# dbolya/yolact

Hardware: NVIDIA H100
Metric: frames/sec @ 550x550 yolact_base (Yolact.forward + Detect + postprocess) (higher is better)
Workload: dtype f16x3 (fp16 hi+lo operand pairs, 3 wgmma passes, fp32 accumulate: fp32-equivalent, parity-tested at 1e-3)

## Files before the change

yolact_b200/csrc/tc_common.cuh:

```cuda
#pragma once
#include <cuda.h>
#include "kernels.cuh"

namespace yb {
namespace tc {

__device__ __forceinline__ uint32_t smem_u32(const void* p) {
  return (uint32_t)__cvta_generic_to_shared(p);
}
__device__ __forceinline__ void mbar_init(uint64_t* bar, uint32_t count) {
  asm volatile("mbarrier.init.shared::cta.b64 [%0], %1;" ::"r"(smem_u32(bar)), "r"(count));
}
__device__ __forceinline__ void mbar_expect_tx(uint64_t* bar, uint32_t bytes) {
  asm volatile("mbarrier.arrive.expect_tx.shared::cta.b64 _, [%0], %1;" ::"r"(smem_u32(bar)), "r"(bytes)
               : "memory");
}
__device__ __forceinline__ bool mbar_try_wait(uint32_t addr, uint32_t parity) {
  uint32_t ok;
  asm volatile(
      "{\n\t"
      ".reg .pred P1;\n\t"
      "mbarrier.try_wait.parity.shared::cta.b64 P1, [%1], %2;\n\t"
      "selp.u32 %0, 1, 0, P1;\n\t"
      "}"
      : "=r"(ok)
      : "r"(addr), "r"(parity)
      : "memory");
  return ok != 0;
}
__device__ __forceinline__ bool mbar_test_wait(uint32_t addr, uint32_t parity) {
  uint32_t ok;
  asm volatile(
      "{\n\t"
      ".reg .pred P1;\n\t"
      "mbarrier.test_wait.parity.shared::cta.b64 P1, [%1], %2;\n\t"
      "selp.u32 %0, 1, 0, P1;\n\t"
      "}"
      : "=r"(ok)
      : "r"(addr), "r"(parity)
      : "memory");
  return ok != 0;
}
__device__ __forceinline__ void mbar_arrive(uint64_t* bar) {
  asm volatile("mbarrier.arrive.shared::cta.b64 _, [%0];" ::"r"(smem_u32(bar)) : "memory");
}
__device__ __forceinline__ void mbar_wait(uint64_t* bar, uint32_t parity) {
  const uint32_t addr = smem_u32(bar);
#ifndef YB_WATCHDOG
  while (!mbar_try_wait(addr, parity)) {
  }
#else
  if (mbar_try_wait(addr, parity)) return;
  const long long t0 = clock64();
  while (!mbar_try_wait(addr, parity)) {
    if (clock64() - t0 > 4000000000ll) asm volatile("trap;");
  }
#endif
}
__device__ __forceinline__ void fence_barrier_init() {
  asm volatile("fence.mbarrier_init.release.cluster;" ::: "memory");
}
__device__ __forceinline__ void tma_prefetch_desc(const void* desc) {
  asm volatile("prefetch.tensormap [%0];" ::"l"(reinterpret_cast<uint64_t>(desc)) : "memory");
}
__device__ __forceinline__ void tma_load_4d(void* smem_dst, const void* desc, uint64_t* bar, int c0,
                                            int c1, int c2, int c3) {
  asm volatile(
      "cp.async.bulk.tensor.4d.shared::cluster.global.mbarrier::complete_tx::bytes"
      " [%0], [%1, {%3, %4, %5, %6}], [%2];" ::"r"(smem_u32(smem_dst)),
      "l"(reinterpret_cast<uint64_t>(desc)), "r"(smem_u32(bar)), "r"(c0), "r"(c1), "r"(c2), "r"(c3)
      : "memory");
}
__device__ __forceinline__ void tma_load_3d(void* smem_dst, const void* desc, uint64_t* bar, int c0,
                                            int c1, int c2) {
  asm volatile(
      "cp.async.bulk.tensor.3d.shared::cluster.global.mbarrier::complete_tx::bytes"
      " [%0], [%1, {%3, %4, %5}], [%2];" ::"r"(smem_u32(smem_dst)),
      "l"(reinterpret_cast<uint64_t>(desc)), "r"(smem_u32(bar)), "r"(c0), "r"(c1), "r"(c2)
      : "memory");
}
__device__ __forceinline__ void tma_store_4d(const void* desc, const void* smem_src, int c0, int c1, int c2, int c3) {
  asm volatile("cp.async.bulk.tensor.4d.global.shared::cta.bulk_group [%0, {%2, %3, %4, %5}], [%1];" ::"l"(
                   reinterpret_cast<uint64_t>(desc)),
               "r"(smem_u32(smem_src)), "r"(c0), "r"(c1), "r"(c2), "r"(c3)
               : "memory");
}
__device__ __forceinline__ void bulk_commit() { asm volatile("cp.async.bulk.commit_group;" ::: "memory"); }
template <int N>
__device__ __forceinline__ void bulk_wait_read() {
  asm volatile("cp.async.bulk.wait_group.read %0;" ::"n"(N) : "memory");
}
__device__ __forceinline__ void bulk_wait_all() { asm volatile("cp.async.bulk.wait_group 0;" ::: "memory"); }
__device__ __forceinline__ void fence_proxy_async() { asm volatile("fence.proxy.async.shared::cta;" ::: "memory"); }
__device__ __forceinline__ void fence_proxy_async_all() { asm volatile("fence.proxy.async;" ::: "memory"); }
__device__ __forceinline__ int ld_acquire_gpu(const int* p) {
  int v;
  asm volatile("ld.acquire.gpu.global.s32 %0, [%1];" : "=r"(v) : "l"(p) : "memory");
  return v;
}
__device__ __forceinline__ void st_release_gpu(int* p, int v) {
  asm volatile("st.release.gpu.global.s32 [%0], %1;" ::"l"(p), "r"(v) : "memory");
}
__device__ __forceinline__ void st_relaxed_gpu(int* p, int v) {
  asm volatile("st.relaxed.gpu.global.s32 [%0], %1;" ::"l"(p), "r"(v) : "memory");
}
__device__ __forceinline__ void red_release_gpu_add(int* p, int v) {
  asm volatile("red.release.gpu.global.add.s32 [%0], %1;" ::"l"(p), "r"(v) : "memory");
}
__device__ __forceinline__ uint4 ldg_nc16(const void* p) {
  uint4 r;
  asm volatile("ld.global.nc.v4.u32 {%0, %1, %2, %3}, [%4];" : "=r"(r.x), "=r"(r.y), "=r"(r.z), "=r"(r.w) : "l"(p));
  return r;
}
__device__ __forceinline__ uint32_t cluster_ctarank() {
  uint32_t r;
  asm volatile("mov.u32 %0, %%cluster_ctarank;" : "=r"(r));
  return r;
}
__device__ __forceinline__ uint32_t cluster_id_x() {
  uint32_t r;
  asm volatile("mov.u32 %0, %%clusterid.x;" : "=r"(r));
  return r;
}
__device__ __forceinline__ uint32_t cluster_nclusters_x() {
  uint32_t r;
  asm volatile("mov.u32 %0, %%nclusterid.x;" : "=r"(r));
  return r;
}
__device__ __forceinline__ void cluster_sync_all() {
  asm volatile("barrier.cluster.arrive.release.aligned;" ::: "memory");
  asm volatile("barrier.cluster.wait.acquire.aligned;" ::: "memory");
}
__device__ __forceinline__ uint32_t mapa_u32(uint32_t smem_cta_addr, uint32_t rank) {
  uint32_t r;
  asm volatile("mapa.shared::cluster.u32 %0, %1, %2;" : "=r"(r) : "r"(smem_cta_addr), "r"(rank));
  return r;
}
__device__ __forceinline__ void mbar_arrive_cluster(uint32_t cluster_addr) {
  asm volatile("mbarrier.arrive.release.cluster.shared::cluster.b64 _, [%0];" ::"r"(cluster_addr) : "memory");
}
__device__ __forceinline__ void tma_load_3d_mc(void* smem_dst, const void* desc, uint64_t* bar, uint16_t mask, int c0, int c1,
                                               int c2) {
  asm volatile(
      "cp.async.bulk.tensor.3d.shared::cluster.global.mbarrier::complete_tx::bytes.multicast::cluster"
      " [%0], [%1, {%3, %4, %5}], [%2], %6;" ::"r"(smem_u32(smem_dst)),
      "l"(reinterpret_cast<uint64_t>(desc)), "r"(smem_u32(bar)), "r"(c0), "r"(c1), "r"(c2), "h"(mask)
      : "memory");
}

__device__ __forceinline__ void wgmma_fence() { asm volatile("wgmma.fence.sync.aligned;" ::: "memory"); }
__device__ __forceinline__ void wgmma_commit() { asm volatile("wgmma.commit_group.sync.aligned;" ::: "memory"); }
template <int N>
__device__ __forceinline__ void wgmma_wait() {
  asm volatile("wgmma.wait_group.sync.aligned %0;" ::"n"(N) : "memory");
}
template <int R>
__device__ __forceinline__ void fence_regs(float* d) {
#pragma unroll
  for (int i = 0; i < R; ++i) asm volatile("" : "+f"(d[i])::"memory");
}
template <int N>
struct Wgmma;
template <>
struct Wgmma<32> {
  __device__ __forceinline__ static void mma(float* d, uint64_t da, uint64_t db, uint32_t scale_d) {
    asm volatile(
        "{\n\t"
        ".reg .pred p;\n\t"
        "setp.ne.b32 p, %18, 0;\n\t"
        "wgmma.mma_async.sync.aligned.m64n32k16.f32.f16.f16 "
        "{"
        "%0, %1, %2, %3, %4, %5, %6, %7, %8, %9, %10, %11, %12, %13, %14, %15 "
        "}, %16, %17, p, 1, 1, 0, 0;\n\t"
        "}"
        : "+f"(d[0]), "+f"(d[1]), "+f"(d[2]), "+f"(d[3]), "+f"(d[4]), "+f"(d[5]), "+f"(d[6]), "+f"(d[7]),
          "+f"(d[8]), "+f"(d[9]), "+f"(d[10]), "+f"(d[11]), "+f"(d[12]), "+f"(d[13]), "+f"(d[14]), "+f"(d[15])
        : "l"(da), "l"(db), "r"(scale_d));
  }
};
template <>
struct Wgmma<64> {
  __device__ __forceinline__ static void mma(float* d, uint64_t da, uint64_t db, uint32_t scale_d) {
    asm volatile(
        "{\n\t"
        ".reg .pred p;\n\t"
        "setp.ne.b32 p, %34, 0;\n\t"
        "wgmma.mma_async.sync.aligned.m64n64k16.f32.f16.f16 "
        "{"
// ... 117 lines not shown
```

yolact_b200/csrc/tc_conv.cu:

```cuda
#include <atomic>
#include <vector>
#include "tc_common.cuh"

namespace yb {

using namespace tc;

namespace {

constexpr int BLOCK_M = 128;
constexpr int BLOCK_K = 64;
constexpr int A_STAGE_BYTES = BLOCK_M * BLOCK_K * 2;
constexpr int MAX_TAPS = 9;
constexpr int MAX_STAGES = 8;

struct alignas(64) TcParams {
  CUtensorMap tmA[4];
  CUtensorMap tmB;
  CUtensorMap tmY;
  CUtensorMap tmR;
  int epi_tma;
  int out_off;
  int res_off;
  int m_tiles, n_tiles;
// ... 3 lines not shown
  float* seg_y[3];
  int pdl;
  int pair;
  int nb;
  int ntaps, kchunks, stages;
  int tap_map[MAX_TAPS], tap_dx[MAX_TAPS], tap_dy[MAX_TAPS];
  int tw, th, tiles_x, tiles_y;
  int Ho, Wo, Cout;
  int a_box_bytes;
  void* y;
  const float* bias;
  const __half* residual;
  long long y_batch_stride;
  long long res_batch_stride;
  int y_pix_stride;
  int y_f32;
  int act;
  int vec_ok;
  int res_after_act;
  int split;
  int cin;
  float out_scale;
  int sk;
  float* sk_ws;
  int* sk_flags;
  int res_direct;
  int bn;
};

__device__ __forceinline__ void mma_bar_sync(int nthreads) { asm volatile("bar.sync 1, %0;" ::"r"(nthreads) : "memory"); }

template <int BN, int MH, int H, bool SPLIT, bool PAIR, int NACC>
__device__ __forceinline__ void mma_tile(float (&acc)[MH][SPLIT ? 2 : 1][NACC], uint8_t* smem, uint64_t* full_bar,
                                         uint64_t* empty_bar, int stages, int stage_bytes, int a_bytes, int b_plane_bytes,
                                         uint32_t& kbg, int nkb, int cw, bool signaller) {
  constexpr int NPL = SPLIT ? 2 : 1;
#pragma unroll
  for (int mh = 0; mh < MH; ++mh)
#pragma unroll
    for (int pl = 0; pl < NPL; ++pl)
#pragma unroll
      for (int i = 0; i < BN / 2; ++i) acc[mh][pl][i] = 0.f;
  auto release = [&](uint32_t s) {
    if (!signaller) return;
    if (PAIR) {
      mbar_arrive_cluster(mapa_u32(smem_u32(&empty_bar[s]), 0));
      mbar_arrive_cluster(mapa_u32(smem_u32(&empty_bar[s]), 1));
    } else {
      mbar_arrive(&empty_bar[s]);
    }
  };
  for (int kb = 0; kb < nkb; ++kb, ++kbg) {
    const uint32_t s = kbg % (uint32_t)stages;
    mbar_wait(&full_bar[s], (kbg / (uint32_t)stages) & 1u);
    const uint32_t sa = smem_u32(smem + (size_t)s * stage_bytes);
    const uint32_t sb = sa + (uint32_t)a_bytes;
    wgmma_fence();
#pragma unroll
    for (int mh = 0; mh < MH; ++mh) {
      const uint32_t half_off = (uint32_t)(cw + mh * H) * (64u * 128u);
      mma_passes<BN, BLOCK_K / 16, SPLIT>(
          acc[mh][0], acc[mh][NPL - 1],
          [&](int pl, int k) { return make_sw128_desc(sa + (uint32_t)(pl * A_STAGE_BYTES) + half_off) + (uint64_t)(2 * k); },
          [&](int pl, int k) { return make_sw128_desc(sb + (uint32_t)(pl * b_plane_bytes)) + (uint64_t)(2 * k); });
    }
    wgmma_commit();
    if (stages == 1) {
      wgmma_wait<0>();
      release(s);
    } else if (kb > 0) {
      wgmma_wait<1>();
      release((kbg - 1) % (uint32_t)stages);
    }
  }
  wgmma_wait<0>();
  if (nkb > 0 && stages > 1) release((kbg - 1) % (uint32_t)stages);
#pragma unroll
  for (int mh = 0; mh < MH; ++mh)
#pragma unroll
    for (int pl = 0; pl < NPL; ++pl) fence_regs<BN / 2>(acc[mh][pl]);
  if (SPLIT) {
#pragma unroll
    for (int mh = 0; mh < MH; ++mh)
#pragma unroll
      for (int i = 0; i < BN / 2; ++i) acc[mh][0][i] = split_combine(acc[mh][0][i], acc[mh][NPL - 1][i]);
  }
}

struct EpiArgs {
  const CUtensorMap* tmY;
  const CUtensorMap* tmR;
  uint64_t* res_full_bar;
  uint8_t* out_base;
  uint8_t* res_base;
  const float* bias;
  const __half* res_g;
  int res_pix_stride;
  uint32_t res_tx;
  int Wo, Cout, n0, x0, y0, b, nchunks, nbuf;
  float out_scale;
};
template <int ACT, bool RES_AFTER, bool SPLIT, int BN, int MH, int H, int NACC>
__device__ __forceinline__ void epi_staged(float (&acc)[MH][SPLIT ? 2 : 1][NACC], const EpiArgs& e, bool has_res_tile,
                                           uint32_t& g, int cw, int ct, int lane, int wq) {
  constexpr int NPL = SPLIT ? 2 : 1;
  const int nthreads = 128 * H;
#pragma unroll
  for (int c = 0; c < BN / 64; ++c) {
    if (c >= e.nchunks) break;
    const uint32_t buf = (e.nbuf == 1) ? 0u : (g & 1u);
    uint8_t* out_tile = e.out_base + buf * (NPL * A_STAGE_BYTES);
    const uint8_t* res_tile = e.res_base + buf * (NPL * A_STAGE_BYTES);
    if (g >= (uint32_t)e.nbuf) {
      if (ct == 0) {
        if (e.nbuf == 1) bulk_wait_read<0>(); else bulk_wait_read<1>();
      }
      mma_bar_sync(nthreads);
    }
    if (has_res_tile) {
      if (ct == 0 && e.nbuf == 2 && c + 1 < e.nchunks) {
        const uint32_t nb = (g + 1) & 1u;
        mbar_expect_tx(&e.res_full_bar[nb], e.res_tx);
#pragma unroll
        for (int pl = 0; pl < NPL; ++pl)
          tma_load_4d(e.res_base + nb * (NPL * A_STAGE_BYTES) + pl * A_STAGE_BYTES, e.tmR, &e.res_full_bar[nb],
                      e.n0 + (c + 1) * 64 + pl * e.Cout, e.x0, e.y0, e.b);
      }
      mbar_wait(&e.res_full_bar[buf], (e.nbuf == 1) ? (g & 1u) : ((g >> 1) & 1u));
    }
    const int nbase = e.n0 + c * 64;
#pragma unroll
    for (int j = 0; j < 8; ++j) {
      const int col = 8 * j + 2 * (lane & 3);
      const float b0 = (e.bias && nbase + col < e.Cout) ? __ldg(e.bias + nbase + col) : 0.f;
      const float b1 = (e.bias && nbase + col + 1 < e.Cout) ? __ldg(e.bias + nbase + col + 1) : 0.f;
#pragma unroll
      for (int mh = 0; mh < MH; ++mh)
#pragma unroll
        for (int h = 0; h < 2; ++h) {
          const int row = (cw + mh * H) * 64 + wq * 16 + (lane >> 2) + 8 * h;
          const int i = (c * 8 + j) * 4 + 2 * h;
          float v0 = scale_bias<SPLIT>(acc[mh][0][i], e.out_scale, b0);
          float v1 = scale_bias<SPLIT>(acc[mh][0][i + 1], e.out_scale, b1);
          if (RES_AFTER) {
            v0 = act_t<ACT>(v0);
            v1 = act_t<ACT>(v1);
          }
          const uint32_t off = sw128_off((uint32_t)row, (uint32_t)j) + (uint32_t)(lane & 3) * 4u;
          if (has_res_tile || e.res_g) {
            __half2 rh, rl;
            if (has_res_tile) {
              rh = *reinterpret_cast<const __half2*>(res_tile + off);
              if (SPLIT) rl = *reinterpret_cast<const __half2*>(res_tile + A_STAGE_BYTES + off);
            } else if (e.x0 + row < e.Wo) {
              const __half* rp = e.res_g + (size_t)row * e.res_pix_stride + c * 64 + col;
              const unsigned int u = __ldcg(reinterpret_cast<const unsigned int*>(rp));
              rh = *reinterpret_cast<const __half2*>(&u);
              if (SPLIT) {
                const unsigned int ul = __ldcg(reinterpret_cast<const unsigned int*>(rp + e.Cout));
                rl = *reinterpret_cast<const __half2*>(&ul);
              }
            } else {
              rh = rl = __floats2half2_rn(0.f, 0.f);
            }
            const float2 f = __half22float2(rh);
            v0 += f.x;
            v1 += f.y;
            if (SPLIT) {
              const float2 fl = lo2_to_f32(rl);
              v0 += fl.x;
              v1 += fl.y;
            }
          }
          if (!RES_AFTER) {
            v0 = act_t<ACT>(v0);
            v1 = act_t<ACT>(v1);
          }
          __half2 hi, lo;
          if (SPLIT) split2_from_f32(v0, v1, hi, lo);
          else hi = f16x2_from_f32(v0, v1);
          *reinterpret_cast<__half2*>(out_tile + off) = hi;
          if (SPLIT) *reinterpret_cast<__half2*>(out_tile + A_STAGE_BYTES + off) = lo;
        }
    }
    fence_proxy_async();
    mma_bar_sync(nthreads);
    if (ct == 0) {
      tma_store_4d(e.tmY, out_tile, nbase, e.x0, e.y0, e.b);
      if (SPLIT) tma_store_4d(e.tmY, out_tile + A_STAGE_BYTES, nbase + e.Cout, e.x0, e.y0, e.b);
      bulk_commit();
      if (has_res_tile && e.nbuf == 1 && c + 1 < e.nchunks) {
        mbar_expect_tx(&e.res_full_bar[0], e.res_tx);
#pragma unroll
        for (int pl = 0; pl < NPL; ++pl)
          tma_load_4d(e.res_base + pl * A_STAGE_BYTES, e.tmR, &e.res_full_bar[0], e.n0 + (c + 1) * 64 + pl * e.Cout, e.x0,
                      e.y0, e.b);
      }
    }
    ++g;
  }
}

template <bool SPLIT, int BN, int MH, int H, int NACC>
__device__ __forceinline__ void epi_staged_act(int act, int raa, float (&acc)[MH][SPLIT ? 2 : 1][NACC], const EpiArgs& e,
                                               bool has_res_tile, uint32_t& g, int cw, int ct, int lane, int wq) {
  switch (act) {
    case ACT_RELU: epi_staged<ACT_RELU, false, SPLIT, BN, MH, H>(acc, e, has_res_tile, g, cw, ct, lane, wq); break;
    case ACT_LEAKY:
      if (raa) epi_staged<ACT_LEAKY, true, SPLIT, BN, MH, H>(acc, e, has_res_tile, g, cw, ct, lane, wq);
      else epi_staged<ACT_LEAKY, false, SPLIT, BN, MH, H>(acc, e, has_res_tile, g, cw, ct, lane, wq);
      break;
    case ACT_TANH: epi_staged<ACT_TANH, false, SPLIT, BN, MH, H>(acc, e, has_res_tile, g, cw, ct, lane, wq); break;
    default: epi_staged<ACT_NONE, false, SPLIT, BN, MH, H>(acc, e, has_res_tile, g, cw, ct, lane, wq); break;
  }
}

struct TileCoord {
  int b, x0, y0, n0;
};
__device__ __forceinline__ TileCoord decode_mn(const TcParams& p, int m, int nt, int BN) {
  TileCoord t;
  const int tx = m % p.tiles_x;
  m /= p.tiles_x;
  const int ty = m % p.tiles_y;
  t.b = m / p.tiles_y;
  t.x0 = tx * p.tw;
  t.y0 = ty * p.th;
  t.n0 = nt * BN;
  return t;
}
template <bool PAIR>
__device__ __forceinline__ TileCoord decode_unit(const TcParams& p, int u, int rank, int BN) {
  const int nt = u % p.n_tiles;
  const int mg = u / p.n_tiles;
  return decode_mn(p, PAIR ? 2 * mg + rank : mg, nt, BN);
}

struct WorkIter {
  int num_kb, num_units, ustep, sk, u;
  long long it, it_hi;
  __device__ __forceinline__ static long long share_lo(long long total, int c, int G) { return total * c / G; }
  __device__ __forceinline__ void init(int sk_, int num_kb_, int num_units_, int unit0, int ustep_) {
    sk = sk_;
    num_kb = num_kb_;
    num_units = num_units_;
    ustep = ustep_;
    u = unit0;
    const long long total = (long long)num_units_ * num_kb_;
    it = share_lo(total, unit0, ustep_);
    it_hi = share_lo(total, unit0 + 1, ustep_);
  }
  __device__ __forceinline__ bool next(int& uu, int& k0, int& k1) {
    if (!sk) {
      if (u >= num_units) return false;
      uu = u;
      k0 = 0;
      k1 = num_kb;
      u += ustep;
      return true;
    }
    if (it >= it_hi) return false;
    uu = (int)(it / num_kb);
    k0 = (int)(it - (long long)uu * num_kb);
    const long long rem = it_hi - it;
    k1 = (rem < (long long)(num_kb - k0)) ? (int)(k0 + rem) : num_kb;
    it += k1 - k0;
    return true;
  }
};

template <int BN, bool PAIR, int H, bool SPLIT>
__global__ void __launch_bounds__(128 * (1 + H), 1)
tc_conv_kernel(const __grid_constant__ TcParams p) {
  constexpr int NPL = SPLIT ? 2 : 1;
  constexpr int MH = 2 / H;
  constexpr int NACC = BN / 2;
  static_assert(MH * NPL * NACC <= 128, "accumulator tile exceeds the register budget");
  constexpr int B_PLANE_BYTES = BN * BLOCK_K * 2;
  constexpr int A_BYTES = NPL * A_STAGE_BYTES;
  constexpr int STAGE_BYTES = A_BYTES + NPL * B_PLANE_BYTES;

  extern __shared__ uint8_t smem_dyn[];
  __shared__ uint64_t full_bar[MAX_STAGES];
  __shared__ uint64_t empty_bar[MAX_STAGES];
  __shared__ uint64_t res_full_bar[2];

  uint8_t* smem = reinterpret_cast<uint8_t*>((reinterpret_cast<uintptr_t>(smem_dyn) + 1023) & ~(uintptr_t)1023);

  const int warp = threadIdx.x >> 5;
  const int lane = threadIdx.x & 31;
  const int stages = p.stages;
  const int num_kb = p.ntaps * p.kchunks;
  const int rank = PAIR ? (int)cluster_ctarank() : 0;
  const int unit0 = PAIR ? (int)cluster_id_x() : (int)blockIdx.x;
  const int ustep = PAIR ? (int)cluster_nclusters_x() : (int)gridDim.x;
  const int num_units = (PAIR ? (p.m_tiles + 1) / 2 : p.m_tiles) * p.n_tiles;

  if (threadIdx.x == 0) {
    for (int s = 0; s < stages; ++s) {
      mbar_init(&full_bar[s], 1);
      mbar_init(&empty_bar[s], (PAIR ? 2 : 1) * H);
    }
    for (int i = 0; i < 2; ++i) mbar_init(&res_full_bar[i], 1);
    fence_barrier_init();
    tma_prefetch_desc(&p.tmB);
    tma_prefetch_desc(&p.tmA[0]);
    if (p.epi_tma) tma_prefetch_desc(&p.tmY);
  }
  __syncthreads();
  if (PAIR) cluster_sync_all();
  uint32_t pre = 0;
  if (p.pdl) {
    asm volatile("griddepcontrol.launch_dependents;" ::: "memory");
    if (!PAIR && !SPLIT && !p.sk && threadIdx.x == 0 && unit0 < num_units) {
      const TileCoord t0 = decode_unit<PAIR>(p, unit0, rank, BN);
      const int npre = min(stages, num_kb);
// ... 119 lines not shown
        e.out_base = out_base;
        e.res_base = res_base;
        e.bias = p.bias;
        e.res_g = (p.res_direct && p.residual) ? p.residual + (size_t)x0 * (size_t)(NPL * p.Cout) + n0 : nullptr;
        e.res_pix_stride = NPL * p.Cout;
        e.res_tx = (uint32_t)p.a_box_bytes * (uint32_t)NPL;
        e.Wo = p.Wo;
        e.Cout = p.Cout;
        e.n0 = n0;
        e.x0 = x0;
        e.y0 = y0;
        e.b = b;
        e.nchunks = nchunks;
        e.nbuf = nbuf;
        e.out_scale = p.out_scale;
        epi_staged_act<SPLIT, BN, MH, H>(p.act, p.res_after_act, acc, e, has_res_tile, g, cw, ct, lane, wq);
      } else {
        const int ncols = min(BN, p.Cout - n0);
        const int raa = p.res_after_act;
#pragma unroll
        for (int j = 0; j < BN / 8; ++j) {
          if (8 * j >= ncols) break;
#pragma unroll
          for (int e2 = 0; e2 < 2; ++e2) {
            const int cl = 8 * j + 2 * (lane & 3) + e2;
            if (cl >= ncols) continue;
            const int n = n0 + cl;
            const float bias_n = p.bias ? __ldg(p.bias + n) : 0.f;
            int act = p.act;
            float* seg_base = nullptr;
            long long seg_bs = 0;
            int seg_ps = 0, seg_c = 0;
            if (p.nseg > 0) {
#pragma unroll
              for (int sg = 0; sg < 3; ++sg)
                if (sg < p.nseg && n >= p.seg_begin[sg] && n < p.seg_end[sg]) {
                  seg_base = p.seg_y[sg];
                  seg_bs = p.seg_bs[sg];
                  seg_ps = p.seg_ps[sg];
                  seg_c = n - p.seg_begin[sg];
                  act = p.seg_act[sg];
                }
            }
#pragma unroll
            for (int mh = 0; mh < MH; ++mh)
#pragma unroll
              for (int h = 0; h < 2; ++h) {
                const int trow = (cw + mh * H) * 64 + wq * 16 + (lane >> 2) + 8 * h;
                const int ty_ = trow / p.tw, tx_ = trow - ty_ * p.tw;
                const int oy = y0 + ty_, ox = x0 + tx_;
                if (trow >= p.tw * p.th || oy >= p.Ho || ox >= p.Wo || b >= p.nb) continue;
                const long long pix = (long long)oy * p.Wo + ox;
                const float a = acc[mh][0][j * 4 + 2 * h + e2];
                float v = scale_bias<SPLIT>(a, p.out_scale, bias_n);
                float rsd = 0.f;
                if (p.residual) {
                  const __half* rp = p.residual + ((long long)b * p.res_batch_stride + pix * p.Cout) * NPL + n;
                  rsd = SPLIT ? split_to_f32(rp[0], rp[p.Cout]) : __half2float(rp[0]);
                }
                if (!raa) v += rsd;
                v = apply_act(v, act);
                if (raa) v += rsd;
                if (p.nseg > 0) {
                  if (seg_base) seg_base[(long long)b * seg_bs + pix * seg_ps + seg_c] = v;
                  continue;
                }
                const long long o = (long long)b * p.y_batch_stride + pix * p.y_pix_stride + n;
                if (p.y_f32) {
                  reinterpret_cast<float*>(p.y)[o] = v;
                } else if (SPLIT) {
                  __half hi, lo;
                  split_f32(v, hi, lo);
                  reinterpret_cast<__half*>(p.y)[o] = hi;
                  reinterpret_cast<__half*>(p.y)[o + p.Cout] = lo;
                } else {
                  reinterpret_cast<__half*>(p.y)[o] = from_f32<__half>(v);
                }
              }
          }
        }
      }
      if (sk_head) {
        mma_bar_sync(128 * H);
        if (ct == 0)
          for (int j = 1; j <= sk_parts; ++j) st_relaxed_gpu(p.sk_flags + 2 * (PAIR ? 2 * (unit0 + j) + rank : unit0 + j), 0);
      }
    }
    if (p.epi_tma && ct == 0) bulk_wait_read<0>();
  }

  __syncthreads();
  if (PAIR) cluster_sync_all();
}

struct ChainLayer {
  int ubase;
  int units;
  int flat;
  int W, H, rows;
  int tw, th, tiles_x, tiles_y;
  int done_off;
  int target;
  int dep_a;
  int dep_r;
  int stride, pad, kh;
};

__host__ __device__ __forceinline__ void chain_rows_of_tile(const ChainLayer& ci, int m, int& r0, int& r1) {
  if (ci.flat) {
    const int lo = m * ci.tw;
    int hi = lo + ci.tw;
    if (hi > ci.rows * ci.W) hi = ci.rows * ci.W;
    r0 = lo / ci.W;
    r1 = (hi - 1) / ci.W;
  } else {
    const int ty = (m / ci.tiles_x) % ci.tiles_y, b = m / (ci.tiles_x * ci.tiles_y);
    int y1 = ty * ci.th + ci.th;
    if (y1 > ci.H) y1 = ci.H;
    r0 = b * ci.H + ty * ci.th;
    r1 = b * ci.H + y1 - 1;
  }
}
__host__ __device__ __forceinline__ void chain_input_rows(const ChainLayer& ci, const ChainLayer& pa, int r0, int r1, int& ra, int& rb) {
  const int b0 = r0 / ci.H, y0 = r0 - b0 * ci.H, b1 = r1 / ci.H, y1 = r1 - b1 * ci.H;
  int lo = y0 * ci.stride - ci.pad, hi = y1 * ci.stride - ci.pad + ci.kh - 1;
  if (lo < 0) lo = 0;
  if (hi > pa.H - 1) hi = pa.H - 1;
  ra = b0 * pa.H + lo;
  rb = b1 * pa.H + hi;
}
__host__ __device__ __forceinline__ void chain_tiles_of_rows(const ChainLayer& pi, int ra, int rb, int& ia, int& ib) {
  if (pi.flat) {
    ia = (ra * pi.W) / pi.tw;
    ib = ((rb + 1) * pi.W - 1) / pi.tw;
  } else {
    const int ba = ra / pi.H, ya = ra - ba * pi.H, bb = rb / pi.H, yb = rb - bb * pi.H;
    ia = (ba * pi.tiles_y + ya / pi.th) * pi.tiles_x;
    ib = (bb * pi.tiles_y + yb / pi.th) * pi.tiles_x + pi.tiles_x - 1;
  }
}

__host__ __device__ constexpr int chain_stages(bool split) { return split ? 3 : 6; }

__device__ __forceinline__ int chain_first_unit(int cta, int ubase, int G) {
  int r = (cta - ubase) % G;
  return r < 0 ? r + G : r;
}

template <bool SPLIT>
__global__ void __launch_bounds__(384, 1)
tc_chain_kernel(const TcParams* __restrict__ layers, const ChainLayer* __restrict__ info, int nl, int* __restrict__ done,
                long long* __restrict__ stats) {
  const long long t_kernel0 = stats ? clock64() : 0;
  long long w0 = 0, w1 = 0;
  constexpr int NPL = SPLIT ? 2 : 1;
  constexpr int B_PLANE_BYTES = 128 * BLOCK_K * 2;
  constexpr int A_BYTES = NPL * A_STAGE_BYTES;
  constexpr int STAGE_BYTES = A_BYTES + NPL * B_PLANE_BYTES;
  constexpr int stages = chain_stages(SPLIT);

  extern __shared__ uint8_t smem_dyn[];
  __shared__ uint64_t full_bar[MAX_STAGES];
  __shared__ uint64_t empty_bar[MAX_STAGES];

  uint8_t* smem = reinterpret_cast<uint8_t*>((reinterpret_cast<uintptr_t>(smem_dyn) + 1023) & ~(uintptr_t)1023);
  const int warp = threadIdx.x >> 5;
  const int lane = threadIdx.x & 31;
  uint8_t* out_base = smem + stages * STAGE_BYTES;
  const int G = (int)gridDim.x;
  const int cta = (int)blockIdx.x;

  if (threadIdx.x == 0) {
    for (int s = 0; s < stages; ++s) {
      mbar_init(&full_bar[s], 1);
      mbar_init(&empty_bar[s], 2);
    }
    fence_barrier_init();
    tma_prefetch_desc(&layers[0].tmB);
    tma_prefetch_desc(&layers[0].tmA[0]);
    tma_prefetch_desc(&layers[0].tmY);
  }
  __syncthreads();

  if (warp < 4) {
    if (warp == 0) {
      uint32_t kbg = 0;
      for (int L = 0; L < nl; ++L) {
        const TcParams& p = layers[L];
        const ChainLayer ci = info[L];
        const int num_kb = p.ntaps * p.kchunks;
        const int bn = p.bn;
        const uint32_t tx_bytes = ((uint32_t)p.a_box_bytes + (uint32_t)(bn * BLOCK_K * 2)) * (uint32_t)NPL;
        if (lane == 0 && L + 1 < nl) {
          tma_prefetch_desc(&layers[L + 1].tmB);
          tma_prefetch_desc(&layers[L + 1].tmA[0]);
        }
        const bool nodeps = (ci.dep_a < 0 && ci.dep_r < 0);
        auto dep_of = [&](int m, int i, const int*& c, int& tgt) -> int {
          int r0, r1;
          chain_rows_of_tile(ci, m, r0, r1);
          int ia = 0, ib = -1, ja = 0, jb = -1, ta = 0, tr = 0;
          const int *ca = done, *cr = done;
          if (ci.dep_a >= 0) {
            const ChainLayer pa = info[ci.dep_a];
            int ra, rb;
            chain_input_rows(ci, pa, r0, r1, ra, rb);
            chain_tiles_of_rows(pa, ra, rb, ia, ib);
            ca = done + pa.done_off;
            ta = pa.target;
          }
          if (ci.dep_r >= 0) {
            const ChainLayer pr = info[ci.dep_r];
            chain_tiles_of_rows(pr, r0, r1, ja, jb);
            cr = done + pr.done_off;
            tr = pr.target;
          }
          const int na = ib - ia + 1, nr = jb - ja + 1;
          if (i < na) {
            c = ca + ia + i;
            tgt = ta;
          } else {
            c = cr + ja + (i - na);
            tgt = tr;
          }
          return na + nr;
        };
        for (int u = chain_first_unit(cta, ci.ubase, G); u < ci.units; u += G) {
          const TileCoord tc_ = decode_unit<false>(p, u, 0, bn);
          bool ready = nodeps;
          for (int kb = 0; kb < num_kb; ++kb, ++kbg) {
            const uint32_t s = kbg % (uint32_t)stages;
            const uint32_t it = kbg / (uint32_t)stages;
            const int tap = kb / p.kchunks;
            const int kc = kb - tap * p.kchunks;
            uint8_t* sa = smem + (size_t)s * STAGE_BYTES;
            uint8_t* sb = sa + A_BYTES;
            if (lane == 0) {
              const long long t0 = stats ? clock64() : 0;
              mbar_wait(&empty_bar[s], (it & 1u) ^ 1u);
              if (stats) w1 += clock64() - t0;
              mbar_expect_tx(&full_bar[s], tx_bytes);
#pragma unroll
              for (int pl = 0; pl < NPL; ++pl)
                tma_load_3d(sb + pl * B_PLANE_BYTES, &p.tmB, &full_bar[s], kc * BLOCK_K + pl * p.cin, tc_.n0, tap);
            }
            if (!ready) {
              const long long tdep0 = stats ? clock64() : 0;
              __syncwarp();
              const int* c = done;
              int tgt = 0;
              const int n = dep_of(u / p.n_tiles, lane, c, tgt);
              for (int i = lane; i < n; i += 32) {
                if (i != lane) dep_of(u / p.n_tiles, i, c, tgt);
#ifdef YB_WATCHDOG
                const long long t0 = clock64();
#endif
                while (ld_acquire_gpu(c) < tgt) {
#ifdef YB_WATCHDOG
                  if (clock64() - t0 > 4000000000ll) asm volatile("trap;");
#endif
                }
              }
              __syncwarp();
              if (stats) w0 += clock64() - tdep0;
              fence_proxy_async_all();
              ready = true;
            }
            if (lane == 0) {
              const CUtensorMap* ma = &p.tmA[p.tap_map[tap]];
              const int ax = tc_.x0 + p.tap_dx[tap], ay = tc_.y0 + p.tap_dy[tap];
#pragma unroll
              for (int pl = 0; pl < NPL; ++pl)
                tma_load_4d(sa + pl * A_STAGE_BYTES, ma, &full_bar[s], kc * BLOCK_K + pl * p.cin, ax, ay, tc_.b);
            }
          }
        }
      }
      if (stats && lane == 0) {
        stats[cta * 8 + 0] = w0;
        stats[cta * 8 + 1] = w1;
      }
    }
  } else {
    const int cw = warp / 4 - 1;
    const int ct = threadIdx.x - 128;
    const int wq = warp & 3;
    const bool signaller = (threadIdx.x & 127) == 0;
    float acc[1][NPL][64];
    int* pending = nullptr;
    auto flush_pending = [&]() {
      const long long t0 = stats ? clock64() : 0;
      bulk_wait_all();
      if (stats) w0 += clock64() - t0;
      fence_proxy_async_all();
      red_release_gpu_add(pending, 1);
      pending = nullptr;
    };
    uint32_t kbg = 0, g = 0;
    for (int L = 0; L < nl; ++L) {
      const TcParams& p = layers[L];
      const int ubase = info[L].ubase, units = info[L].units, done_off = info[L].done_off;
      const int num_kb = p.ntaps * p.kchunks;
      const int n_tiles = p.n_tiles;
      const int bn = p.bn;
      for (int u = chain_first_unit(cta, ubase, G); u < units; u += G) {
        const TileCoord tc_ = decode_unit<false>(p, u, 0, bn);
        if (ct == 0 && pending &&
            !mbar_test_wait(smem_u32(&full_bar[kbg % (uint32_t)stages]), (kbg / (uint32_t)stages) & 1u))
          flush_pending();
        if (bn == 128)
          mma_tile<128, 1, 2, SPLIT, false>(acc, smem, full_bar, empty_bar, stages, STAGE_BYTES, A_BYTES, B_PLANE_BYTES, kbg,
                                            num_kb, cw, signaller);
        else
          mma_tile<64, 1, 2, SPLIT, false>(acc, smem, full_bar, empty_bar, stages, STAGE_BYTES, A_BYTES, B_PLANE_BYTES, kbg,
                                           num_kb, cw, signaller);
        if (ct == 0 && pending) flush_pending();
        EpiArgs e;
        e.tmY = &p.tmY;
        e.tmR = &p.tmR;
        e.res_full_bar = nullptr;
        e.out_base = out_base;
        e.res_base = nullptr;
        e.bias = p.bias;
        e.res_g = p.residual ? p.residual + (size_t)tc_.x0 * (size_t)(NPL * p.Cout) + tc_.n0 : nullptr;
        e.res_pix_stride = NPL * p.Cout;
        e.res_tx = 0;
        e.Wo = p.Wo;
        e.Cout = p.Cout;
        e.n0 = tc_.n0;
        e.x0 = tc_.x0;
        e.y0 = tc_.y0;
        e.b = tc_.b;
        e.nchunks = bn / 64;
        e.nbuf = SPLIT ? 1 : 2;
        e.out_scale = p.out_scale;
        if (bn == 128) epi_staged_act<SPLIT, 128, 1, 2>(p.act, p.res_after_act, acc, e, false, g, cw, ct, lane, wq);
        else epi_staged_act<SPLIT, 64, 1, 2>(p.act, p.res_after_act, acc, e, false, g, cw, ct, lane, wq);
        if (ct == 0) pending = done + done_off + u / n_tiles;
      }
    }
    if (ct == 0) {
      if (pending) flush_pending();
      bulk_wait_read<0>();
      if (stats) {
        stats[cta * 8 + 4] = w0;
        stats[cta * 8 + 6] = clock64() - t_kernel0;
      }
    }
  }
  __syncthreads();
}

int floordiv(int a, int b) { return (a >= 0) ? a / b : -((-a + b - 1) / b); }

}

int device_sms() {
  static std::atomic<int> cached[64] = {};
  int dev = 0;
  YB_CHECK_CUDA(cudaGetDevice(&dev));
  int n = cached[dev & 63].load();
  if (n <= 0) {
    YB_CHECK_CUDA(cudaDeviceGetAttribute(&n, cudaDevAttrMultiProcessorCount, dev));
    cached[dev & 63].store(n);
  }
  return n;
}

typedef CUresult (*PFN_encodeTiled)(CUtensorMap*, CUtensorMapDataType, cuuint32_t, void*, const cuuint64_t*,
                                    const cuuint64_t*, const cuuint32_t*, const cuuint32_t*,
                                    CUtensorMapInterleave, CUtensorMapSwizzle, CUtensorMapL2promotion,
                                    CUtensorMapFloatOOBfill);

namespace {
PFN_encodeTiled get_encode_fn() {
  static PFN_encodeTiled fn = nullptr;
  if (fn) return fn;
  void* ptr = nullptr;
  cudaDriverEntryPointQueryResult qres;
  YB_CHECK_CUDA(cudaGetDriverEntryPoint("cuTensorMapEncodeTiled", &ptr, cudaEnableDefault, &qres));
  YB_REQUIRE(qres == cudaDriverEntryPointSuccess && ptr, "cuTensorMapEncodeTiled not available from the driver");
  fn = reinterpret_cast<PFN_encodeTiled>(ptr);
  return fn;
}

}

void tc::encode_map_f16(CUtensorMap* map, const void* base, int rank, const uint64_t* dims, const uint64_t* strides_bytes,
                const uint32_t* box, int swizzle_bytes) {
  cuuint64_t gdim[5];
  cuuint64_t gstr[5];
  cuuint32_t bx[5];
  cuuint32_t es[5];
  for (int i = 0; i < rank; ++i) {
    gdim[i] = dims[i];
    bx[i] = box[i];
    es[i] = 1;
    YB_REQUIRE(box[i] >= 1 && box[i] <= 256, "tensor map: box dim out of range");
  }
  for (int i = 0; i + 1 < rank; ++i) {
    gstr[i] = strides_bytes[i];
    YB_REQUIRE(strides_bytes[i] % 16 == 0, "tensor map: stride must be a multiple of 16 bytes");
  }
  YB_REQUIRE((reinterpret_cast<uintptr_t>(base) & 15) == 0, "tensor map: base must be 16-byte aligned");
  CUresult r = get_encode_fn()(map, CU_TENSOR_MAP_DATA_TYPE_FLOAT16, (cuuint32_t)rank, const_cast<void*>(base),
                               gdim, gstr, bx, es, CU_TENSOR_MAP_INTERLEAVE_NONE,
                               swizzle_bytes == 64 ? CU_TENSOR_MAP_SWIZZLE_64B : CU_TENSOR_MAP_SWIZZLE_128B,
                               CU_TENSOR_MAP_L2_PROMOTION_L2_256B,
                               CU_TENSOR_MAP_FLOAT_OOB_FILL_NONE);
  if (r != CUDA_SUCCESS)
    throw Error(YB_ERR_CUDA, "cuTensorMapEncodeTiled failed with CUresult " + std::to_string((int)r));
}


struct TcConvPlan {
  TcParams prm;
  int split = 0;
  int sk = 0;
  int BN = 128;
  int pair = 0;
  int epi_groups = 1;
  int pdl_friendly = 0;
  int chain = 0;
  int flat = 0;
  int B = 0, Ho = 0, Wo = 0;
  int Hi = 0, Wi = 0, stride = 1, pad = 0, KH = 1;
  dim3 grid;
  size_t smem_bytes = 0;
};

bool tc_conv_supported(const ConvProblem& p) {
  if (p.x_nchw_f32) return false;
  if (p.Cin % BLOCK_K != 0) return false;
  if (p.KH * p.KW > MAX_TAPS) return false;
  if (p.stride != 1 && p.stride != 2) return false;
  if (p.Cout < 1) return false;
  return true;
}

static void choose_tile(int Wov, int Hov, int& best_tw, int& best_th) {
  best_tw = 1;
  best_th = 1;
  double best_eff = -1.0;
  for (int tw = 1; tw <= std::min(Wov, 128); ++tw) {
    int th = std::min(Hov, 128 / tw);
    if (th < 1) continue;
    if (tw > 256 || th > 256) continue;
    long long tiles = (long long)ceil_div(Wov, tw) * ceil_div(Hov, th);
    double eff = (double)Wov * Hov / ((double)tiles * 128.0);
    if (eff > best_eff + 1e-9 || (eff > best_eff - 1e-9 && tw > best_tw)) {
      best_eff = eff;
      best_tw = tw;
      best_th = th;
    }
  }
}

void tc_chain_debug_deps(int B, int Hin, int Win, int k, int stride, int pad, int producer_flat, int m, int32_t* out) {
  YB_REQUIRE(B >= 1 && Hin >= 1 && Win >= 1 && (k == 1 || k == 3) && (stride == 1 || stride == 2) && pad >= 0 && out,
             "chain_debug_deps: bad argument");
  const int Ho = (Hin + 2 * pad - k) / stride + 1, Wo = (Win + 2 * pad - k) / stride + 1;
  YB_REQUIRE(Ho >= 1 && Wo >= 1, "chain_debug_deps: empty output");
  auto layer = [&](int flat, int H, int W, int s, int p, int kh) {
    ChainLayer c = {};
    c.flat = flat;
    c.W = W;
    c.H = H;
    c.rows = B * H;
    const int Wov = flat ? B * H * W : W, Hov = flat ? 1 : H;
    choose_tile(Wov, Hov, c.tw, c.th);
    c.tiles_x = ceil_div(Wov, c.tw);
    c.tiles_y = ceil_div(Hov, c.th);
    c.stride = s;
    c.pad = p;
    c.kh = kh;
    return c;
  };
  const ChainLayer ci = layer((k == 1 && stride == 1 && pad == 0) ? 1 : 0, Ho, Wo, stride, pad, k);
  const ChainLayer pa = layer(producer_flat ? 1 : 0, Hin, Win, 1, 0, 1);
  const int cm = ci.tiles_x * ci.tiles_y * (ci.flat ? 1 : B), pm = pa.tiles_x * pa.tiles_y * (pa.flat ? 1 : B);
  YB_REQUIRE(m >= 0 && m < cm, "chain_debug_deps: tile out of range");
  int r0, r1, ra, rb, ia, ib;
  chain_rows_of_tile(ci, m, r0, r1);
  chain_input_rows(ci, pa, r0, r1, ra, rb);
  chain_tiles_of_rows(pa, ra, rb, ia, ib);
  const int32_t v[14] = {ci.flat, ci.tw, ci.th, ci.tiles_x, ci.tiles_y, cm, pa.flat, pa.tw, pa.th, pa.tiles_x, pa.tiles_y, pm, ia, ib};
  for (int i = 0; i < 14; ++i) out[i] = v[i];
}

TcConvPlan* tc_conv_plan_create(const ConvProblem& p, const __half* w_packed, const TcTiling& want) {
  YB_REQUIRE(tc_conv_supported(p), "tc_conv: unsupported problem");
  YB_REQUIRE(p.Ho == (p.H + 2 * p.pad - p.KH) / p.stride + 1, "tc_conv: bad Ho");
  YB_REQUIRE(p.Wo == (p.W + 2 * p.pad - p.KW) / p.stride + 1, "tc_conv: bad Wo");
  auto* plan = new TcConvPlan();
  TcParams& q = plan->prm;
  memset(&q, 0, sizeof(q));
  const int s = p.stride;
// ... 270 lines not shown
  if (plan->epi_groups == 2) {
    if constexpr (NPL * BN / 2 <= 128) launch_bn<BN, PAIR, 2, SPLIT>(plan, stream);
    else YB_REQUIRE(false, "tc_conv: N tile too wide for two MMA warpgroups");
  } else {
    if constexpr (NPL * BN <= 128) launch_bn<BN, PAIR, 1, SPLIT>(plan, stream);
    else YB_REQUIRE(false, "tc_conv: N tile too wide for one MMA warpgroup");
  }
}

template <bool SPLIT>
static void launch_s(const TcConvPlan* plan, cudaStream_t stream) {
  if (plan->pair) {
    switch (plan->BN) {
      case 256: launch_h<256, true, SPLIT>(plan, stream); break;
      case 128: launch_h<128, true, SPLIT>(plan, stream); break;
      case 64: launch_h<64, true, SPLIT>(plan, stream); break;
      default: YB_REQUIRE(false, "tc_conv: bad BN for a CTA pair");
    }
  } else {
    switch (plan->BN) {
      case 256: launch_h<256, false, SPLIT>(plan, stream); break;
      case 128: launch_h<128, false, SPLIT>(plan, stream); break;
      case 64: launch_h<64, false, SPLIT>(plan, stream); break;
      case 32: launch_h<32, false, SPLIT>(plan, stream); break;
      default: YB_REQUIRE(false, "tc_conv: bad BN");
    }
  }
}

struct TcChain {
  int nl = 0, split = 0, grid = 0, n_done = 0;
  size_t smem_bytes = 0;
  TcParams* d_layers = nullptr;
  ChainLayer* d_info = nullptr;
  int* d_done = nullptr;
  long long* d_stats = nullptr;
};

bool tc_conv_plan_chainable(const TcConvPlan* pl) {
  const TcParams& q = pl->prm;
  return (pl->BN == 128 || pl->BN == 64) && !pl->pair && pl->epi_groups == 2 && !pl->sk && !pl->pdl_friendly && q.epi_tma &&
         q.nseg == 0 && q.Cout % pl->BN == 0 && (!q.residual || q.res_direct) && (q.act == ACT_RELU || q.act == ACT_NONE || q.act == ACT_LEAKY);
}

TcChain* tc_chain_create(const std::vector<const TcConvPlan*>& plans, const std::vector<int>& dep_a, const std::vector<int>& dep_r) {
  YB_REQUIRE(!plans.empty() && plans.size() == dep_a.size() && plans.size() == dep_r.size(), "tc_chain: empty chain");
  const TcConvPlan* p0 = plans[0];
  std::vector<TcParams> lp;
  std::vector<ChainLayer> li;
  int ubase = 0, done_off = 0;
  for (size_t i = 0; i < plans.size(); ++i) {
    const TcConvPlan* pl = plans[i];
    YB_REQUIRE(tc_conv_plan_chainable(pl), "tc_chain: plan not chainable");
    YB_REQUIRE(pl->split == p0->split, "tc_chain: the layers of a chain share one precision mode");
    YB_REQUIRE(pl->B == p0->B, "tc_chain: the layers of a chain share one batch size");
    YB_REQUIRE(dep_a[i] < (int)i && dep_r[i] < (int)i, "tc_chain: dependencies point backwards");
    YB_REQUIRE(dep_r[i] < 0 || (plans[dep_r[i]]->Ho == pl->Ho && plans[dep_r[i]]->Wo == pl->Wo), "tc_chain: residual geometry");
    YB_REQUIRE(dep_a[i] < 0 || (plans[dep_a[i]]->Ho == pl->Hi && plans[dep_a[i]]->Wo == pl->Wi), "tc_chain: input geometry");
    ChainLayer c = {};
    c.ubase = ubase;
    c.units = pl->prm.m_tiles * pl->prm.n_tiles;
    c.flat = pl->flat;
    c.W = pl->Wo;
    c.H = pl->Ho;
    c.rows = pl->B * pl->Ho;
    c.tw = pl->prm.tw;
    c.th = pl->prm.th;
    c.tiles_x = pl->prm.tiles_x;
    c.tiles_y = pl->prm.tiles_y;
    c.done_off = done_off;
    c.target = pl->prm.n_tiles;
    c.dep_a = dep_a[i];
    c.dep_r = dep_r[i];
    c.stride = pl->stride;
    c.pad = pl->pad;
    c.kh = pl->KH;
    ubase += c.units;
    done_off += pl->prm.m_tiles;
    lp.push_back(pl->prm);
    li.push_back(c);
  }
  auto* ch = new TcChain();
  ch->nl = (int)plans.size();
  ch->split = p0->split;
  ch->n_done = done_off;
  {
    const int npl = p0->split ? 2 : 1;
    ch->smem_bytes = (size_t)chain_stages(p0->split != 0) * npl * (A_STAGE_BYTES + 128 * BLOCK_K * 2) +
                     (size_t)(p0->split ? 1 : 2) * npl * A_STAGE_BYTES + 1024;
  }
  const int sms = device_sms();
  ch->grid = std::min(sms, ubase);
  try {
    YB_CHECK_CUDA(cudaMalloc(&ch->d_layers, lp.size() * sizeof(TcParams)));
    YB_CHECK_CUDA(cudaMalloc(&ch->d_info, li.size() * sizeof(ChainLayer)));
    YB_CHECK_CUDA(cudaMalloc(&ch->d_done, (size_t)done_off * sizeof(int)));
    YB_CHECK_CUDA(cudaMemcpy(ch->d_layers, lp.data(), lp.size() * sizeof(TcParams), cudaMemcpyHostToDevice));
    YB_CHECK_CUDA(cudaMemcpy(ch->d_info, li.data(), li.size() * sizeof(ChainLayer), cudaMemcpyHostToDevice));
  } catch (...) {
    tc_chain_destroy(ch);
    throw;
  }
  return ch;
}
void tc_chain_destroy(TcChain* ch) {
  if (!ch) return;
  cudaFree(ch->d_layers);
  cudaFree(ch->d_info);
  cudaFree(ch->d_done);
  cudaFree(ch->d_stats);
  delete ch;
}
int tc_chain_layers(const TcChain* ch) { return ch->nl; }

template <bool SPLIT>
static void launch_chain_t(const TcChain* ch, cudaStream_t stream) {
  static PerDeviceOnce attr;
  if (attr.first())
    YB_CHECK_CUDA(cudaFuncSetAttribute(tc_chain_kernel<SPLIT>, cudaFuncAttributeMaxDynamicSharedMemorySize,
                                       (int)ch->smem_bytes));
  cudaLaunchConfig_t cfg = {};
  cfg.gridDim = dim3((unsigned)ch->grid);
  cfg.blockDim = dim3(384);
  cfg.dynamicSmemBytes = ch->smem_bytes;
  cfg.stream = stream;
  cudaLaunchAttribute at[1];
  at[0].id = cudaLaunchAttributeCooperative;
  at[0].val.cooperative = 1;
  cfg.attrs = at;
  cfg.numAttrs = 1;
  YB_CHECK_CUDA(cudaLaunchKernelEx(&cfg, tc_chain_kernel<SPLIT>, (const TcParams*)ch->d_layers, (const ChainLayer*)ch->d_info,
                                   ch->nl, ch->d_done, ch->d_stats));
}

void tc_chain_print_stats(TcChain* ch, const char* name) {
  const int G = ch->grid;
  YB_CHECK_CUDA(cudaMalloc(&ch->d_stats, (size_t)G * 8 * sizeof(long long)));
  YB_CHECK_CUDA(cudaMemset(ch->d_stats, 0, (size_t)G * 8 * sizeof(long long)));
  launch_tc_chain(ch, 0, nullptr);
  YB_CHECK_CUDA(cudaDeviceSynchronize());
  std::vector<long long> hs((size_t)G * 8);
  YB_CHECK_CUDA(cudaMemcpy(hs.data(), ch->d_stats, hs.size() * sizeof(long long), cudaMemcpyDeviceToHost));
  cudaFree(ch->d_stats);
  ch->d_stats = nullptr;
  double avg[8] = {}, mx[8] = {};
  for (int c = 0; c < G; ++c)
    for (int k = 0; k < 8; ++k) {
      avg[k] += (double)hs[(size_t)c * 8 + k] / G;
      mx[k] = std::max(mx[k], (double)hs[(size_t)c * 8 + k]);
    }
  const double tot = avg[6] > 0 ? avg[6] : 1.0;
  fprintf(stderr,
          "[yolact_b200] chain stats %s: kernel %.0f kcyc/CTA; share of it spent waiting (avg over CTAs / max): producer deps %.1f%% / %.1f%%, "
          "producer ring slot %.1f%%, store completion before a signal %.1f%% / %.1f%%\n",
          name, tot / 1e3, 100 * avg[0] / tot, 100 * mx[0] / tot, 100 * avg[1] / tot, 100 * avg[4] / tot, 100 * mx[4] / tot);
}

bool tc_chain_graph_ok(const TcChain* ch) {
  static std::atomic<int> cached{-1};
  if (cached.load() >= 0) return cached.load() != 0;
  bool ok = false;
  cudaStream_t s = nullptr;
  cudaGraph_t g = nullptr;
  cudaGraphExec_t ge = nullptr;
  if (cudaStreamCreateWithFlags(&s, cudaStreamNonBlocking) == cudaSuccess) {
    if (cudaStreamBeginCapture(s, cudaStreamCaptureModeThreadLocal) == cudaSuccess) {
      try {
        launch_tc_chain(ch, s, nullptr);
      } catch (const Error&) {
      }
      if (cudaStreamEndCapture(s, &g) == cudaSuccess && g && cudaGraphInstantiate(&ge, g, 0) == cudaSuccess)
        ok = (cudaGraphLaunch(ge, s) == cudaSuccess) && (cudaStreamSynchronize(s) == cudaSuccess);
    }
  }
  if (ge) cudaGraphExecDestroy(ge);
  if (g) cudaGraphDestroy(g);
  if (s) cudaStreamDestroy(s);
  cudaGetLastError();
  cached.store(ok ? 1 : 0);
  return ok;
}
void launch_tc_chain(const TcChain* ch, cudaStream_t stream, LaunchCounter* lc) {
  YB_CHECK_CUDA(cudaMemsetAsync(ch->d_done, 0, (size_t)ch->n_done * sizeof(int), stream));
  if (ch->split) launch_chain_t<true>(ch, stream); else launch_chain_t<false>(ch, stream);
  YB_CHECK_LAUNCH();
  if (lc) lc->n++;
}

void launch_tc_conv(const TcConvPlan* plan, cudaStream_t stream, LaunchCounter* lc) {
  if (plan->split) launch_s<true>(plan, stream); else launch_s<false>(plan, stream);
  YB_CHECK_LAUNCH();
  if (lc) lc->n++;
}

}
```

Before: 506.5.

## Signal tile completion right after epilogue and make residual loads branchless

Drops the deferred pending-signal scheme, in which a tile's completion counter was only released after the next tile's MMA or when the producer stalled. Thread 0 now waits for its bulk stores and releases the dependency counter right after each epilogue. Downstream consumers see results sooner, but the MMA warpgroup now blocks on store completion before starting its next tile. The epilogue's global residual load also becomes branchless: it clamps the row, loads unconditionally and zeroes out-of-range values. Epilogue timing is added to the stats output.

Measured after the change: 520.4 (median of 6 runs). 2.8% higher.

```diff
diff --git a/yolact_b200/csrc/tc_common.cuh b/yolact_b200/csrc/tc_common.cuh
--- a/yolact_b200/csrc/tc_common.cuh
+++ b/yolact_b200/csrc/tc_common.cuh
@@ -21,19 +21,6 @@
       "{\n\t"
       ".reg .pred P1;\n\t"
       "mbarrier.try_wait.parity.shared::cta.b64 P1, [%1], %2;\n\t"
-      "selp.u32 %0, 1, 0, P1;\n\t"
-      "}"
-      : "=r"(ok)
-      : "r"(addr), "r"(parity)
-      : "memory");
-  return ok != 0;
-}
-__device__ __forceinline__ bool mbar_test_wait(uint32_t addr, uint32_t parity) {
-  uint32_t ok;
-  asm volatile(
-      "{\n\t"
-      ".reg .pred P1;\n\t"
-      "mbarrier.test_wait.parity.shared::cta.b64 P1, [%1], %2;\n\t"
       "selp.u32 %0, 1, 0, P1;\n\t"
       "}"
       : "=r"(ok)
diff --git a/yolact_b200/csrc/tc_conv.cu b/yolact_b200/csrc/tc_conv.cu
--- a/yolact_b200/csrc/tc_conv.cu
+++ b/yolact_b200/csrc/tc_conv.cu
@@ -179,16 +179,17 @@
             if (has_res_tile) {
               rh = *reinterpret_cast<const __half2*>(res_tile + off);
               if (SPLIT) rl = *reinterpret_cast<const __half2*>(res_tile + A_STAGE_BYTES + off);
-            } else if (e.x0 + row < e.Wo) {
-              const __half* rp = e.res_g + (size_t)row * e.res_pix_stride + c * 64 + col;
-              const unsigned int u = __ldcg(reinterpret_cast<const unsigned int*>(rp));
+            } else {
+              const bool in = e.x0 + row < e.Wo;
+              const __half* rp = e.res_g + (long long)(in ? row : e.Wo - 1 - e.x0) * e.res_pix_stride + c * 64 + col;
+              unsigned int u = __ldcg(reinterpret_cast<const unsigned int*>(rp));
+              u = in ? u : 0u;
               rh = *reinterpret_cast<const __half2*>(&u);
               if (SPLIT) {
-                const unsigned int ul = __ldcg(reinterpret_cast<const unsigned int*>(rp + e.Cout));
+                unsigned int ul = __ldcg(reinterpret_cast<const unsigned int*>(rp + e.Cout));
+                ul = in ? ul : 0u;
                 rl = *reinterpret_cast<const __half2*>(&ul);
               }
-            } else {
-              rh = rl = __floats2half2_rn(0.f, 0.f);
             }
             const float2 f = __half22float2(rh);
             v0 += f.x;
@@ -614,7 +615,7 @@
 tc_chain_kernel(const TcParams* __restrict__ layers, const ChainLayer* __restrict__ info, int nl, int* __restrict__ done,
                 long long* __restrict__ stats) {
   const long long t_kernel0 = stats ? clock64() : 0;
-  long long w0 = 0, w1 = 0;
+  long long w0 = 0, w1 = 0, w_epi = 0;
   constexpr int NPL = SPLIT ? 2 : 1;
   constexpr int B_PLANE_BYTES = 128 * BLOCK_K * 2;
   constexpr int A_BYTES = NPL * A_STAGE_BYTES;
@@ -749,15 +750,6 @@
     const int wq = warp & 3;
     const bool signaller = (threadIdx.x & 127) == 0;
     float acc[1][NPL][64];
-    int* pending = nullptr;
-    auto flush_pending = [&]() {
-      const long long t0 = stats ? clock64() : 0;
-      bulk_wait_all();
-      if (stats) w0 += clock64() - t0;
-      fence_proxy_async_all();
-      red_release_gpu_add(pending, 1);
-      pending = nullptr;
-    };
     uint32_t kbg = 0, g = 0;
     for (int L = 0; L < nl; ++L) {
       const TcParams& p = layers[L];
@@ -767,16 +759,12 @@
       const int bn = p.bn;
       for (int u = chain_first_unit(cta, ubase, G); u < units; u += G) {
         const TileCoord tc_ = decode_unit<false>(p, u, 0, bn);
-        if (ct == 0 && pending &&
-            !mbar_test_wait(smem_u32(&full_bar[kbg % (uint32_t)stages]), (kbg / (uint32_t)stages) & 1u))
-          flush_pending();
         if (bn == 128)
           mma_tile<128, 1, 2, SPLIT, false>(acc, smem, full_bar, empty_bar, stages, STAGE_BYTES, A_BYTES, B_PLANE_BYTES, kbg,
                                             num_kb, cw, signaller);
         else
           mma_tile<64, 1, 2, SPLIT, false>(acc, smem, full_bar, empty_bar, stages, STAGE_BYTES, A_BYTES, B_PLANE_BYTES, kbg,
                                            num_kb, cw, signaller);
-        if (ct == 0 && pending) flush_pending();
         EpiArgs e;
         e.tmY = &p.tmY;
         e.tmR = &p.tmR;
@@ -796,15 +784,23 @@
         e.nchunks = bn / 64;
         e.nbuf = SPLIT ? 1 : 2;
         e.out_scale = p.out_scale;
+        const long long t_epi = stats ? clock64() : 0;
         if (bn == 128) epi_staged_act<SPLIT, 128, 1, 2>(p.act, p.res_after_act, acc, e, false, g, cw, ct, lane, wq);
         else epi_staged_act<SPLIT, 64, 1, 2>(p.act, p.res_after_act, acc, e, false, g, cw, ct, lane, wq);
-        if (ct == 0) pending = done + done_off + u / n_tiles;
+        if (stats) w_epi += clock64() - t_epi;
+        if (ct == 0) {
+          const long long t0 = stats ? clock64() : 0;
+          bulk_wait_all();
+          if (stats) w0 += clock64() - t0;
+          fence_proxy_async_all();
+          red_release_gpu_add(done + done_off + u / n_tiles, 1);
+        }
       }
     }
     if (ct == 0) {
-      if (pending) flush_pending();
       bulk_wait_read<0>();
       if (stats) {
+        stats[cta * 8 + 2] = w_epi;
         stats[cta * 8 + 4] = w0;
         stats[cta * 8 + 6] = clock64() - t_kernel0;
       }
@@ -1381,8 +1377,10 @@
   const double tot = avg[6] > 0 ? avg[6] : 1.0;
   fprintf(stderr,
           "[yolact_b200] chain stats %s: kernel %.0f kcyc/CTA; share of it spent waiting (avg over CTAs / max): producer deps %.1f%% / %.1f%%, "
-          "producer ring slot %.1f%%, store completion before a signal %.1f%% / %.1f%%\n",
-          name, tot / 1e3, 100 * avg[0] / tot, 100 * mx[0] / tot, 100 * avg[1] / tot, 100 * avg[4] / tot, 100 * mx[4] / tot);
+          "producer ring slot %.1f%%, store completion before a signal %.1f%% / %.1f%%; MMA warpgroups in epilogue work "
+          "%.1f%% / %.1f%%\n",
+          name, tot / 1e3, 100 * avg[0] / tot, 100 * mx[0] / tot, 100 * avg[1] / tot, 100 * avg[4] / tot, 100 * mx[4] / tot,
+          100 * avg[2] / tot, 100 * mx[2] / tot);
 }
 
 bool tc_chain_graph_ok(const TcChain* ch) {
```
